# NickTravers/NeuralNetworkLibrary

Hardware: AMD Instinct MI355X
Metric: ResNet-34 224x224 training throughput (Learner.train1minibatch, fwd+loss+bwd+optimizer) (higher is better)
Workload: dtype f32; 1 GPU; DogsCats ResNet-34 classifier, 224x224, bs=64 per GPU, SGD momentum 0.9, fp32; global_batch=64, image_size=224, parallelism=dp1

## Files before the change

### include/nnl.h

```cpp
#ifndef NNL_H_
#define NNL_H_

#include <stddef.h>
#include <stdint.h>

#ifdef __cplusplus
extern "C" {
#endif

typedef enum {
  NNL_OK = 0,
  NNL_ERR_INVALID_ARG = -1,
  NNL_ERR_HIP = -2,
  NNL_ERR_UNSUPPORTED = -3,
  NNL_ERR_WORKSPACE = -4
} nnl_status_t;

int nnl_version(void);
const char* nnl_last_error(void);
int nnl_reload_env(void);

enum { NNL_PROF_CONV_FWD = 0, NNL_PROF_CONV_DGRAD = 1, NNL_PROF_CONV_WGRAD = 2, NNL_PROF_EMBDOT = 3,
       NNL_PROF_TABULAR = 4, NNL_PROF_RETINA_LOSS = 5, NNL_PROF_LSTM = 6, NNL_PROF_SOFTMAX_CE = 7,
       NNL_PROF_ELEMENTWISE = 8, NNL_PROF_GEMM = 9, NNL_PROF_OPTIM = 10, NNL_PROF_KINDS = 11 };
// ... 49 lines not shown
int nnl_wino_filter_multi(const nnl_wino_desc_t* desc, const int32_t* block_desc, int64_t n_blocks, void* stream);
int nnl_conv2d_fwd_pre(const float* x, const float* w, const float* bias, float* y, const nnl_conv_geom_t* g, int relu,
                       void* workspace, size_t workspace_bytes, int32_t* tile_counters, float* bn_partials, const float* bn_pivot,
                       int32_t* bn_rows, const float* u, void* stream);
int nnl_conv2d_dgrad_pre(const float* dy, const float* wt, float* dx, const nnl_conv_geom_t* g, const float* addend,
                         void* workspace, size_t workspace_bytes, int32_t* tile_counters, const float* u, void* stream);
size_t nnl_debug_conv_wino_workspace_bytes(int N, int H, int W, int C, int K);
int nnl_debug_conv_wino_fwd(const float* x, const float* filt, const float* bias, const float* add, float* y, void* ws,
                            size_t ws_bytes, int32_t* counters, long n_counters, float* bn_part, const float* bn_pivot, int N,
                            int H, int W, int C, int K, int relu, int flip, void* stream);
size_t nnl_debug_conv_wino2_workspace_bytes(int N, int H, int W, int C, int K);
int nnl_debug_conv_wino2_fwd(const float* x, const float* filt, const float* bias, const float* add, float* y, void* ws,
                            size_t ws_bytes, int32_t* counters, long n_counters, float* bn_part, const float* bn_pivot, int N,
                            int H, int W, int C, int K, int relu, int flip, void* stream);
int nnl_debug_conv_plan_times(int N, int H, int W, int C, int K, double* out);
size_t nnl_conv2d_wgrad_workspace_bytes(const nnl_conv_geom_t* g);
int nnl_conv2d_wgrad(const float* x, const float* dy, float* dw, const nnl_conv_geom_t* g, void* workspace,
                     size_t workspace_bytes, void* stream);
size_t nnl_colsum_workspace_bytes(int64_t rows, int64_t cols);
int nnl_sum_tensors(const float* const* src, int n, float* out, int64_t numel, void* stream);
int nnl_colsum(const float* a, float* out, int64_t rows, int64_t cols, void* workspace, size_t workspace_bytes,
               void* stream);
int nnl_relu_gate_colsum(const float* dy, const float* y, float* g, float* colsum, int64_t rows, int64_t cols, void* workspace,
                         size_t workspace_bytes, void* stream);
int nnl_act_gate_colsum(const float* dy, const float* y, float* g, float* colsum, int64_t rows, int64_t cols, int act,
                        void* workspace, size_t workspace_bytes, void* stream);

size_t nnl_bn_workspace_bytes(int64_t rows, int64_t C);
int nnl_bn_fwd(const float* x, const float* gamma, const float* beta, const float* residual, float* y,
               float* save_mean, float* save_invstd, float* running_mean, float* running_var, int64_t rows,
// ... 148 lines not shown
```

### neuralnetworklibrary_amd/_lib.py

```python
import ctypes as C
import os

import torch

_HERE = os.path.dirname(os.path.abspath(__file__))
LIB_PATH = os.environ.get('NNL_LIB_PATH') or os.path.join(_HERE, 'libnnl_hip.so')

if not os.path.exists(LIB_PATH):
    raise ImportError(
        f"{LIB_PATH} not found: build it with `python -c 'import __graft_entry__ as g; g.build()'` "
        "(or `make -C neuralnetworklibrary_amd/csrc`). There is no CPU fallback for the HIP hot path.")

lib = C.CDLL(LIB_PATH)

c_p = C.c_void_p
i32, i64, f32, f64 = C.c_int32, C.c_int64, C.c_float, C.c_double
sz = C.c_size_t


class ConvGeom(C.Structure):
    _fields_ = [('N', i32), ('H', i32), ('W', i32), ('C', i32), ('K', i32), ('R', i32), ('S', i32),
                ('stride', i32), ('pad', i32), ('P', i32), ('Q', i32)]


# ... 13 lines not shown
    'nnl_embdotbias_bwd_workspace_bytes': (sz, [i64]),
    'nnl_embdotbias_bwd': (C.c_int, [c_p, c_p, c_p, c_p, c_p, c_p, c_p, c_p, c_p, i64, i64, i64, i64, C.c_int,
                                     f32, f32, c_p, sz, c_p]),
    'nnl_conv2d_fwd_workspace_bytes': (sz, [C.POINTER(ConvGeom)]),
    'nnl_conv2d_dgrad_workspace_bytes': (sz, [C.POINTER(ConvGeom)]),
    'nnl_conv2d_tile_counters': (i64, []),
    'nnl_conv2d_wino_preferred': (C.c_int, [C.POINTER(ConvGeom), C.c_int]),
    'nnl_wino_filter_multi': (C.c_int, [c_p, c_p, i64, c_p]),
    'nnl_conv2d_fwd_pre': (C.c_int, [c_p, c_p, c_p, c_p, C.POINTER(ConvGeom), C.c_int, c_p, sz, c_p, c_p, c_p, C.POINTER(i32), c_p, c_p]),
    'nnl_conv2d_dgrad_pre': (C.c_int, [c_p, c_p, c_p, C.POINTER(ConvGeom), c_p, c_p, sz, c_p, c_p, c_p]),
    'nnl_debug_conv_wino_workspace_bytes': (sz, [C.c_int] * 5),
    'nnl_debug_conv_wino_fwd': (C.c_int, [c_p] * 6 + [sz, c_p, C.c_long, c_p, c_p] + [C.c_int] * 7 + [c_p]),
    'nnl_debug_conv_wino2_workspace_bytes': (sz, [C.c_int] * 5),
    'nnl_debug_conv_wino2_fwd': (C.c_int, [c_p] * 6 + [sz, c_p, C.c_long, c_p, c_p] + [C.c_int] * 7 + [c_p]),
    'nnl_debug_conv_plan_times': (C.c_int, [C.c_int] * 5 + [C.POINTER(C.c_double)]),
    'nnl_conv2d_fwd': (C.c_int, [c_p, c_p, c_p, c_p, C.POINTER(ConvGeom), C.c_int, c_p, sz, c_p, c_p, c_p, C.POINTER(i32), c_p]),
    'nnl_conv2d_weight_transpose': (C.c_int, [c_p, c_p, C.c_int, C.c_int, C.c_int, C.c_int, c_p]),
    'nnl_conv2d_weight_transpose_multi': (C.c_int, [c_p, c_p, i64, f64, c_p]),
    'nnl_conv2d_dgrad': (C.c_int, [c_p, c_p, c_p, C.POINTER(ConvGeom), c_p, c_p, sz, c_p, c_p]),
    'nnl_conv2d_wgrad_workspace_bytes': (sz, [C.POINTER(ConvGeom)]),
    'nnl_conv2d_wgrad': (C.c_int, [c_p, c_p, c_p, C.POINTER(ConvGeom), c_p, sz, c_p]),
    'nnl_colsum_workspace_bytes': (sz, [i64, i64]),
    'nnl_colsum': (C.c_int, [c_p, c_p, i64, i64, c_p, sz, c_p]),
    'nnl_relu_gate_colsum': (C.c_int, [c_p, c_p, c_p, c_p, i64, i64, c_p, sz, c_p]),
    'nnl_conv2d_fwd_add_up2': (C.c_int, [c_p, c_p, c_p, c_p, c_p, C.POINTER(ConvGeom), c_p]),
    'nnl_upsample2_bwd': (C.c_int, [c_p, c_p, i64, i64, i64, i64, c_p]),
    'nnl_act_gate_colsum': (C.c_int, [c_p, c_p, c_p, c_p, i64, i64, C.c_int, c_p, sz, c_p]),
    'nnl_maxpool2d_fwd': (C.c_int, [c_p, c_p, c_p, i64, i64, i64, i64, i64, i64, C.c_int, C.c_int, C.c_int, c_p]),
    'nnl_maxpool2d_bwd': (C.c_int, [c_p, c_p, c_p, i64, i64, i64, i64, i64, i64, C.c_int, C.c_int, C.c_int, c_p]),
    'nnl_sum_tensors': (C.c_int, [c_p, C.c_int, c_p, i64, c_p]),
# ... 123 lines not shown
```

### neuralnetworklibrary_amd/csrc/igemm.h

```cpp
#pragma once
#include "nnl_common.h"

typedef float f32x16 __attribute__((ext_vector_type(16)));
typedef float f32x4 __attribute__((ext_vector_type(4)));

struct IgemmRowkParams {
  const float* a;
  const float* b;
  float* y;
  const float* bias;
  const float* add;
  int N, H, W, C;
  int P, Q;
  int R, S, stride, pad;
  int M, Nc, Kg;
  int relu;
  int grid_m, grid_n;
};

struct IgemmKmajorParams {
  const float* a;
  const float* b;
  float* y;
  int N, H, W, C;
  int P, Q;
  int R, S, stride, pad;
  int Mc, Nc;
  long Kp;
  int splits, k_per_split;
  int grid_m, grid_n;
};

int nnl_internal_gemm_nt(const float* a, const float* b, float* y, const float* bias, const float* add, int M, int N,
                         int K, int relu, hipStream_t s);
int nnl_internal_gemm_nt_splitk(const float* a, const float* b, float* y_slabs, int M, int N, int K, int splits, hipStream_t s);
size_t nnl_internal_gemm_tn_workspace_bytes(int Mc, int Nc, long Kp);
int nnl_internal_gemm_tn(const float* a, const float* b, float* y, int Mc, int Nc, long Kp, void* ws, size_t ws_bytes,
                         hipStream_t s);

__device__ __forceinline__ int nnl_xcd_remap(int bid, int nblk) {
  const int q = nblk >> 3, r = nblk & 7;
  const int xcd = bid & 7, idx = bid >> 3;
  const int base = (xcd < r) ? xcd * (q + 1) : r * (q + 1) + (xcd - r) * q;
  return base + idx;
}
```

### neuralnetworklibrary_amd/csrc/wino2.hip

```cpp
#include "wino.h"
#include "wino_filter.h"
#include "igemm_taps.h"
#include <algorithm>

namespace {

constexpr int kCUs = 256;

template <int POL>
__device__ __forceinline__ f32x4 buf_load4_spol(__amdgpu_buffer_rsrc_t rsrc, unsigned voff, unsigned soff) {
  const i32x4 v = __builtin_bit_cast(i32x4, __builtin_amdgcn_raw_buffer_load_b128(rsrc, (int)voff, (int)soff, POL));
  return __builtin_bit_cast(f32x4, v);
}

struct Wino2Params {
  const float* a;
  const float* b;
  float* y;
  const float* bias;
  const float* add;
  unsigned a_bytes, b_bytes;
  int H, W, C, H2, W2;
  int ch;
  int prio;
  int M4;
  unsigned mg_W2, mg_H2;
  int Nc;
// ... 2 lines not shown
  int bal, main_ks, n_main_tiles, tail_slices, tail_row0;
  float* main_out; long main_slab_stride;
  float* tail_out; long tail_slab_stride;
  int* tile_counters;
  float* bn_part; const float* bn_pivot;
  int pos_cs;
};

__global__ void wino2_filter_kernel(const float* __restrict__ w, float* __restrict__ u, long KC, int C, int flip) {
  const long i = (long)blockIdx.x * blockDim.x + threadIdx.x;
  if (i >= KC) return;
  const long c = i % C, k = i / C;
  wino2_filter_item(w + k * 9 * C + c, u + k * 16 * C + c, C, flip);
}

template <int BK, int OCC, bool POS = false>
__global__ __launch_bounds__(256, OCC) void wino2_kernel(const Wino2Params p) {
  constexpr int BM = 64, BN = 64, BKP = BK + 4, KC = BK / 4, RPP = 256 / KC, PA = BM / RPP, PB = BN / RPP;
  __shared__ __attribute__((aligned(16))) float lds[2][(BM + BN) * BKP];
  const int tid = threadIdx.x, lane = tid & 63, wave = tid >> 6, wm = wave >> 1, wn = wave & 1;
  int logical, kslice = 0, nslices = 1, row0 = 0;
  bool in_tail = false;
  if (p.bal) {
    const int nmb = p.n_main_tiles * p.main_ks;
    if ((int)blockIdx.x < nmb) {
      const int u = nnl_xcd_remap(blockIdx.x, nmb);
      logical = u / p.main_ks;
      kslice = u - logical * p.main_ks;
      nslices = p.main_ks;
    } else {
      const int tb = (int)blockIdx.x - nmb;
      const int t = tb / p.tail_slices;
      kslice = tb - t * p.tail_slices;
      logical = p.n_main_tiles + t;
      nslices = p.tail_slices;
      if (nslices > 1) { row0 = p.tail_row0; in_tail = true; }
    }
  } else {
    logical = nnl_xcd_remap(blockIdx.x, gridDim.x);
  }
  const bool partial = nslices > 1;
  const int tile_m = logical / p.grid_n, tile_n = logical - tile_m * p.grid_n;
  const int m0 = tile_m * BM, n0 = tile_n * BN;
  const int kc = tid % KC, lrow = tid / KC;
  auto qdiv = [](int n, unsigned mg) { return mg ? (int)__umulhi((unsigned)n, mg) : n; };
  const __amdgpu_buffer_rsrc_t ra_src = __builtin_amdgcn_make_buffer_rsrc(const_cast<float*>(p.a), 0, (int)p.a_bytes, 0x00020000);
  const __amdgpu_buffer_rsrc_t rb_src = __builtin_amdgcn_make_buffer_rsrc(const_cast<float*>(p.b), 0, (int)p.b_bytes, 0x00020000);

  int a_off[PA];
  unsigned rmask[PA], cmask[PA];
#pragma unroll
  for (int i = 0; i < PA; ++i) {
    const int m = m0 + lrow + i * RPP;
    const bool valid = m < p.M4;
    const int mm = valid ? m : 0;
    const int l2 = qdiv(mm, p.mg_W2), j = mm - l2 * p.W2;
    const int n = qdiv(l2, p.mg_H2), ii = l2 - n * p.H2;
    a_off[i] = (((n * p.H + 2 * ii - 1) * p.W + 2 * j - 1) * p.C + kc * 4) * 4;
    unsigned rm = 0, cm = 0;
    if (valid) {
      for (int a = 0; a < 4; ++a) if ((unsigned)(2 * ii - 1 + a) < (unsigned)p.H) rm |= 1u << a;
      for (int a = 0; a < 4; ++a) if ((unsigned)(2 * j - 1 + a) < (unsigned)p.W) cm |= 1u << a;
    }
    rmask[i] = rm; cmask[i] = cm;
  }
  unsigned b_off[PB];
#pragma unroll
  for (int i = 0; i < PB; ++i) {
    const int nr = n0 + lrow + i * RPP;
    b_off[i] = nr < p.Nc ? (unsigned)(nr * 16 * p.C + kc * 4) * 4u : 0xFFFFFFFFu;
  }
  unsigned v00[PA], v01[PA], v10[PA], v11[PA], b_tap = 0;
  float sr = 1.f, sc = 1.f;
  auto set_pos = [&](int t) {
    const int xi = t >> 2, nu = t & 3;
    const int ra_ = xi, rb_ = xi < 2 ? 2 : 1;
    const int ca = nu, cb = nu < 2 ? 2 : 1;
    sr = xi == 1 ? 1.f : -1.f;
    sc = nu == 1 ? 1.f : -1.f;
    b_tap = (unsigned)(t * p.C) * 4u;
    const int wc = p.W * p.C * 4, c4 = p.C * 4;
#pragma unroll
    for (int i = 0; i < PA; ++i) {
      const bool ra_ok = (rmask[i] >> ra_) & 1u, rb_ok = (rmask[i] >> rb_) & 1u;
      const bool ca_ok = (cmask[i] >> ca) & 1u, cb_ok = (cmask[i] >> cb) & 1u;
      v00[i] = (ra_ok && ca_ok) ? (unsigned)(a_off[i] + ra_ * wc + ca * c4) : 0xFFFFFFFFu;
// ... 15 lines not shown
  float sr_ld = 1.f, sc_ld = 1.f;
  auto store_tile = [&](int buf) {
    float* As = lds[buf];
    float* Bs = As + BM * BKP;
#pragma unroll
    for (int i = 0; i < PA; ++i) {
      f32x4 v;
#pragma unroll
      for (int e = 0; e < 4; ++e)
        v[e] = __builtin_fmaf(sr_ld, __builtin_fmaf(sc_ld, r11[i][e], r10[i][e]), __builtin_fmaf(sc_ld, r01[i][e], r00[i][e]));
      *reinterpret_cast<f32x4*>(As + (lrow + i * RPP) * BKP + kc * 4) = v;
    }
#pragma unroll
    for (int i = 0; i < PB; ++i) *reinterpret_cast<f32x4*>(Bs + (lrow + i * RPP) * BKP + kc * 4) = rb[i];
  };
  const int frag_off = (lane & 31) * BKP + (lane >> 5) * 4;
  auto compute = [&](int buf, f32x16& acc) {
    const float* As = lds[buf] + wm * 32 * BKP + frag_off;
    const float* Bs = lds[buf] + BM * BKP + wn * 32 * BKP + frag_off;
    f32x4 fa[BK / 8], fb[BK / 8];
#pragma unroll
    for (int kk = 0; kk < BK / 8; ++kk) {
      fa[kk] = *reinterpret_cast<const f32x4*>(As + kk * 8);
      fb[kk] = *reinterpret_cast<const f32x4*>(Bs + kk * 8);
    }
#pragma unroll
    for (int kk = 0; kk < BK / 8; ++kk)
#pragma unroll
      for (int t = 0; t < 4; ++t) acc = __builtin_amdgcn_mfma_f32_32x32x2f32(fa[kk][t], fb[kk][t], acc, 0, 0, 0);
  };

  f32x16 y00, y01, y10, y11, tm;
#pragma unroll
  for (int e = 0; e < 16; ++e) { tm[e] = 0.f; }
  if constexpr (!POS) {
#pragma unroll
    for (int e = 0; e < 16; ++e) { y00[e] = 0.f; y01[e] = 0.f; y10[e] = 0.f; y11[e] = 0.f; }
  }
  const int csteps = p.C / BK, nk_all = 16 * csteps, cpc = p.ch / BK, per_chunk = 16 * cpc;
  if constexpr (POS) {
    const int t_pos = kslice / p.pos_cs, sub = kslice - t_pos * p.pos_cs, nkb = csteps / p.pos_cs;
    set_pos(t_pos);
    sr_ld = sr; sc_ld = sc;
    const int cb0 = sub * nkb * BK;
    load_tile(cb0);
    store_tile(0);
    __syncthreads();
    int cur = 0;
    for (int kt = 0; kt < nkb; ++kt) {
      if (kt + 1 < nkb) load_tile(cb0 + (kt + 1) * BK);
      __builtin_amdgcn_sched_barrier(0);
      compute(cur, tm);
      __builtin_amdgcn_sched_barrier(0);
      if (kt + 1 < nkb) store_tile(cur ^ 1);
      __syncthreads();
      cur ^= 1;
    }
  }
  int kt0 = 0, nk = nk_all;
  if (POS) nk = 0;
  else if (partial) {
    const int per = (nk_all + nslices - 1) / nslices;
    kt0 = kslice * per;
    nk = min(per, nk_all - kt0);
    if (nk < 0) nk = 0;
  }
  const int kend = kt0 + nk;
  int chunk_nx = kt0 / per_chunk, t_nx = (kt0 - chunk_nx * per_chunk) / cpc, cs_nx = kt0 - chunk_nx * per_chunk - t_nx * cpc;
  int c_nx = chunk_nx * p.ch + cs_nx * BK;
  int t_cur = t_nx, cs_cur = cs_nx;
  auto advance = [&]() {
    if (++cs_nx == cpc) {
      cs_nx = 0;
      if (++t_nx == 16) { t_nx = 0; ++chunk_nx; }
      set_pos(t_nx);
    }
// ... 35 lines not shown
      }
      if (k10 != 0.f) {
#pragma unroll
        for (int e = 0; e < 16; ++e) y10[e] = __builtin_fmaf(k10, tm[e], y10[e]);
      }
      if (k11 != 0.f) {
#pragma unroll
        for (int e = 0; e < 16; ++e) y11[e] = __builtin_fmaf(k11, tm[e], y11[e]);
      }
#pragma unroll
      for (int e = 0; e < 16; ++e) tm[e] = 0.f;
      cs_cur = 0; t_cur = (t_cur + 1) & 15;
    }
  }

  const int col_l = lane & 31, row_h = (lane >> 5) * 4;
  constexpr int kSc1 = 1 << 4;
  if constexpr (POS) {
    __shared__ int ticket;
    const long sstride = p.main_slab_stride;
    const __amdgpu_buffer_rsrc_t rs = __builtin_amdgcn_make_buffer_rsrc(p.main_out, 0, (int)((long)nslices * sstride * 4), 0x00020000);
    const int cl = n0 + wn * 32 + col_l;
#pragma unroll
    for (int e = 0; e < 16; ++e) {
      const int row = m0 + wm * 32 + (e & 3) + 8 * (e >> 2) + row_h;
      const long off = (long)kslice * sstride + (long)row * p.Nc + cl;
      const bool ok = row < p.M4 && cl < p.Nc;
      __builtin_amdgcn_raw_buffer_store_b32(__float_as_uint(tm[e]), rs, ok ? (int)(off * 4) : -1, 0, kSc1);
    }
    asm volatile("s_waitcnt vmcnt(0)" ::: "memory");
    __syncthreads();
    if (tid == 0) ticket = __hip_atomic_fetch_add(&p.tile_counters[logical], 1, __ATOMIC_RELAXED, __HIP_MEMORY_SCOPE_AGENT);
    __syncthreads();
    if (ticket != nslices - 1) return;
    if (tid == 0) __hip_atomic_store(&p.tile_counters[logical], 0, __ATOMIC_RELAXED, __HIP_MEMORY_SCOPE_AGENT);
    float fs1[4] = {0.f, 0.f, 0.f, 0.f}, fs2[4] = {0.f, 0.f, 0.f, 0.f};
    const int c4 = n0 + (tid & 15) * 4, cs = p.pos_cs;
    const int wrow = p.W * p.Nc;
    auto item_off = [&](int k4, bool& ok) {
      const int row = m0 + (tid >> 4) + 16 * k4;
      ok = row < p.M4 && c4 < p.Nc;
      return ok ? (unsigned)(((long)row * p.Nc + c4) * 4) : 0xFFFFFFFFu;
    };
    auto finish_item = [&](int k4, f32x4 (&m)[16]) {
      const int row = m0 + (tid >> 4) + 16 * k4;
      f32x4 r0[4], r1[4];
#pragma unroll
      for (int xi = 0; xi < 4; ++xi) {
        r0[xi] = (m[xi * 4 + 0] + m[xi * 4 + 1]) + m[xi * 4 + 2];
        r1[xi] = (m[xi * 4 + 1] - m[xi * 4 + 2]) + m[xi * 4 + 3];
      }
      f32x4 out[4];
      out[0] = (r0[0] + r0[1]) + r0[2];
      out[1] = (r1[0] + r1[1]) + r1[2];
      out[2] = (r0[1] - r0[2]) + r0[3];
      out[3] = (r1[1] - r1[2]) + r1[3];
      const int l2 = qdiv(row, p.mg_W2), j = row - l2 * p.W2;
      const int n = qdiv(l2, p.mg_H2), ii = l2 - n * p.H2;
      const long ob = (((long)n * p.H + 2 * ii) * p.W + 2 * j) * p.Nc + c4;
      const bool h1 = 2 * ii + 1 < p.H, w1 = 2 * j + 1 < p.W;
#pragma unroll
      for (int h = 0; h < 4; ++h) {
        if (((h >> 1) && !h1) || ((h & 1) && !w1)) continue;
        f32x4 v = out[h];
        const long o = ob + (h >> 1) * wrow + (h & 1) * p.Nc;
        if (p.bias) v += *reinterpret_cast<const f32x4*>(p.bias + c4);
        if (p.add) v += *reinterpret_cast<const f32x4*>(p.add + o);
        if (p.relu == 1) { v[0] = fmaxf(v[0], 0.f); v[1] = fmaxf(v[1], 0.f); v[2] = fmaxf(v[2], 0.f); v[3] = fmaxf(v[3], 0.f); }
        *reinterpret_cast<f32x4*>(p.y + o) = v;
        if (p.bn_part) {
          const f32x4 pv = *reinterpret_cast<const f32x4*>(p.bn_pivot + c4);
#pragma unroll
          for (int e = 0; e < 4; ++e) { const float d = v[e] - pv[e]; fs1[e] += d; fs2[e] += d * d; }
        }
      }
    };
#pragma unroll 1
    for (int k4 = 0; k4 < 4; ++k4) {
      bool ok_a;
      const unsigned oa = item_off(k4, ok_a);
      if (!ok_a) continue;
      f32x4 ma[16];
#pragma unroll
      for (int t = 0; t < 16; ++t) ma[t] = buf_load4_spol<kSc1>(rs, oa, (unsigned)((long)(t * cs) * sstride * 4));
      for (int sl = 1; sl < cs; ++sl) {
#pragma unroll
        for (int t0 = 0; t0 < 16; t0 += 8) {
          f32x4 pa[8];
#pragma unroll
          for (int t = 0; t < 8; ++t) pa[t] = buf_load4_spol<kSc1>(rs, oa, (unsigned)((long)((t0 + t) * cs + sl) * sstride * 4));
#pragma unroll
          for (int t = 0; t < 8; ++t) ma[t0 + t] += pa[t];
        }
      }
      finish_item(k4, ma);
    }
    if (p.bn_part) {
      __syncthreads();
      float* red = &lds[0][0];
#pragma unroll
      for (int e = 0; e < 4; ++e) {
        red[(((tid >> 4) * 64) + (tid & 15) * 4 + e) * 2 + 0] = fs1[e];
        red[(((tid >> 4) * 64) + (tid & 15) * 4 + e) * 2 + 1] = fs2[e];
      }
      __syncthreads();
      if (tid < 64 && n0 + tid < p.Nc) {
        float a = 0.f, b = 0.f;
        for (int r = 0; r < 16; ++r) { a += red[(r * 64 + tid) * 2]; b += red[(r * 64 + tid) * 2 + 1]; }
        p.bn_part[((long)tile_m * p.Nc + n0 + tid) * 2 + 0] = a;
        p.bn_part[((long)tile_m * p.Nc + n0 + tid) * 2 + 1] = b;
      }
    }
    return;
  }
  if (partial) {
    __shared__ int ticket;
    float* const base = in_tail ? p.tail_out : p.main_out;
    const long sstride = in_tail ? p.tail_slab_stride : p.main_slab_stride;
    const __amdgpu_buffer_rsrc_t rs = __builtin_amdgcn_make_buffer_rsrc(base, 0, (int)((long)nslices * sstride * 4), 0x00020000);
    const int cl = n0 + wn * 32 + col_l;
#pragma unroll
    for (int e = 0; e < 16; ++e) {
      const int row = m0 + wm * 32 + (e & 3) + 8 * (e >> 2) + row_h;
      const long off = (long)kslice * sstride + (long)(row - row0) * 4 * p.Nc + cl;
      const bool ok = row < p.M4 && cl < p.Nc;
      __builtin_amdgcn_raw_buffer_store_b32(__float_as_uint(y00[e]), rs, ok ? (int)(off * 4) : -1, 0, kSc1);
      __builtin_amdgcn_raw_buffer_store_b32(__float_as_uint(y01[e]), rs, ok ? (int)((off + p.Nc) * 4) : -1, 0, kSc1);
      __builtin_amdgcn_raw_buffer_store_b32(__float_as_uint(y10[e]), rs, ok ? (int)((off + 2 * p.Nc) * 4) : -1, 0, kSc1);
      __builtin_amdgcn_raw_buffer_store_b32(__float_as_uint(y11[e]), rs, ok ? (int)((off + 3 * p.Nc) * 4) : -1, 0, kSc1);
// ... 102 lines not shown
    __syncthreads();
    if (tid < 64 && n0 + tid < p.Nc) {
      float a = 0.f, b = 0.f;
      for (int r = 0; r < 16; ++r) { a += red[(r * 64 + tid) * 2]; b += red[(r * 64 + tid) * 2 + 1]; }
      p.bn_part[((long)tile_m * p.Nc + n0 + tid) * 2 + 0] = a;
      p.bn_part[((long)tile_m * p.Nc + n0 + tid) * 2 + 1] = b;
    }
  }
}

struct W2Plan {
  int bk, on, main_ks, n_main_tiles, tail_slices, tail_row0;
  size_t main_floats, tail_floats;
  double t_us;
  int pos_cs;
};

double w2_pos_cost(long T, long M4, int Nc, int C, int cs) {
  const double a = 0.363, b = 0.490, tfix = 4.0;
  const long occ = 4, nwg = T * 16 * cs, I = (C / 32) / cs;
  const long nb = nnl_cdiv(nwg, (long)kCUs);
  const double c = (double)(nb < occ ? nb : occ);
  const double slab_b = 2.0 * 16 * cs * (double)M4 * Nc * 4;
  return nb * I * (b + a / c) + tfix * nb / c + slab_b / 11.7e6 + (3.0 + 1.5 * cs) + 4.0;
}

double w2_cost(long T, long gn, long M4, int Nc, long I, int bk, int ks, int S, W2Plan* out) {
  const double a = bk == 32 ? 0.363 : 0.226, b = bk == 32 ? 0.490 : 0.243, tfix = bk == 32 ? 12.3 : 15.0;
  const long occ = bk == 16 ? 4 : 3;
  long n_main = ((T * ks / kCUs) * kCUs / ks / gn) * gn;
  if (n_main > T) n_main = T;
  const long tail = T - n_main;
  if (tail == 0 && S > 1) return -1.0;
  const long m = nnl_cdiv(n_main * ks, (long)kCUs), q = nnl_cdiv(tail * S, (long)kCUs);
  const long W = m * nnl_cdiv(I, (long)ks) + q * nnl_cdiv(I, (long)S), nb = m + q;
  const double c = (double)(nb < occ ? nb : occ);
  const long row0 = (n_main / gn) * 64 < M4 ? (n_main / gn) * 64 : M4;
  const double main_b = ks > 1 ? (2.0 * ks + 1) * row0 * 4 * Nc * 4 : 0;
  const double tail_b = (S > 1 && tail) ? (2.0 * S + 1) * (M4 - row0) * 4 * Nc * 4 : 0;
// ... 24 lines not shown
        W2Plan cand{};
        const double t = w2_cost(T, gn, M4, Nc, I, bk, ks, S, &cand);
        if (t < 0) break;
        if (f_S > 0 && balance && cand.n_main_tiles < T && S != f_S) continue;
        if (t < best_t) { best_t = t; best = cand; best.t_us = t; }
      }
    }
  }
  if (best_t == 1e300) {
    best.t_us = w2_cost(T, gn, M4, Nc, 16L * (C / 16), 16, 1, 1, &best);
    best_t = best.t_us;
  }
  const int e_pos = NNL_ENV_INT("NNL_WINO2_POS", -1);
  if (e_pos != 0 && (balance || e_pos > 0) && C % 32 == 0) {
    const int csteps = C / 32;
    double pt = 1e300; int pcs = 0;
    for (int cs = 1; cs <= 8; cs *= 2) {
      if (csteps % cs != 0 || (csteps / cs < 2 && cs > 1)) break;
      if (e_pos > 0 && cs != e_pos && csteps % e_pos == 0) continue;
      const size_t fl = (size_t)16 * cs * M4 * Nc;
      if (fl * sizeof(float) >= (1UL << 31)) break;
      const double t = w2_pos_cost(T, M4, Nc, C, cs);
      if (t < pt) { pt = t; pcs = cs; }
    }
    if (pcs && (e_pos > 0 || pt < best_t)) {
      best = W2Plan{};
      best.bk = 32; best.on = 1; best.main_ks = 16 * pcs; best.n_main_tiles = (int)T; best.tail_slices = 1; best.tail_row0 = (int)M4;
      best.main_floats = (size_t)16 * pcs * M4 * Nc; best.tail_floats = 0; best.t_us = pt; best.pos_cs = pcs;
    }
  }
  return best;
}

size_t align4(size_t floats) { return (floats + 3) & ~(size_t)3; }

long quads(int N, int H, int W) { return (long)N * ((H + 1) / 2) * ((W + 1) / 2); }

}

bool nnl_wino2_ok(int N, int H, int W, int Cin, int Nc, int R, int S, int stride, int pad) {
  if (R != 3 || S != 3 || stride != 1 || pad != 1 || W < 2 || H < 2 || Cin % 16 != 0 || Nc % 4 != 0) return false;
  const long a_b = (long)N * H * W * Cin * 4, b_b = (long)Nc * 16 * Cin * 4, y_b = (long)N * H * W * Nc * 4;
  if ((quads(N, H, W) + 128) * (long)std::max((W + 1) / 2, (H + 1) / 2) >= (1L << 32)) return false;
// ... 38 lines not shown
  const long T = (long)p.grid_m * p.grid_n;
  W2Plan pl = wino2_plan(M4, q.Nc, q.Cin);
  if (pl.on && (tile_counters == nullptr || T > n_counters || ws_bytes < (u_floats + pl.main_floats + pl.tail_floats) * sizeof(float) ||
                pl.main_floats * sizeof(float) >= (1UL << 31) || pl.tail_floats * sizeof(float) >= (1UL << 31))) {
    if (pl.pos_cs) {
      const int bk = q.Cin % 32 == 0 ? 32 : 16;
      w2_cost(T, p.grid_n, M4, q.Nc, 16L * (q.Cin / bk), bk, 1, 1, &pl);
      pl.pos_cs = 0;
    }
    pl.on = 0;
  }
  unsigned grid = (unsigned)T;
  if (pl.pos_cs) {
    p.bal = 1; p.main_ks = pl.main_ks; p.n_main_tiles = pl.n_main_tiles; p.tail_slices = 1; p.tail_row0 = (int)M4;
    p.main_out = u + u_floats; p.main_slab_stride = M4 * q.Nc; p.tile_counters = tile_counters; p.pos_cs = pl.pos_cs;
    grid = (unsigned)(T * pl.main_ks);
    hipLaunchKernelGGL((wino2_kernel<32, 4, true>), dim3(grid), dim3(256), 0, s, p);
    NNL_CHECK_LAUNCH();
    return NNL_OK;
  }
  if (pl.on) {
    p.bal = 1; p.main_ks = pl.main_ks; p.n_main_tiles = pl.n_main_tiles; p.tail_slices = pl.tail_slices; p.tail_row0 = pl.tail_row0;
    p.main_out = u + u_floats; p.main_slab_stride = (long)pl.tail_row0 * 4 * q.Nc;
    p.tail_out = p.main_out + pl.main_floats; p.tail_slab_stride = (long)(M4 - pl.tail_row0) * 4 * q.Nc;
    p.tile_counters = tile_counters;
    grid = (unsigned)(pl.n_main_tiles * pl.main_ks + (T - pl.n_main_tiles) * pl.tail_slices);
  }
  if (pl.bk == 32) hipLaunchKernelGGL((wino2_kernel<32, 3>), dim3(grid), dim3(256), 0, s, p);
  else hipLaunchKernelGGL((wino2_kernel<16, 4>), dim3(grid), dim3(256), 0, s, p);
  NNL_CHECK_LAUNCH();
  return NNL_OK;
}

extern "C" size_t nnl_debug_conv_wino2_workspace_bytes(int N, int H, int W, int C, int K) { return nnl_wino2_workspace_bytes(N, H, W, C, K); }
extern "C" int nnl_debug_conv_wino2_fwd(const float* x, const float* w, const float* bias, const float* add, float* y, void* ws,
                                        size_t ws_bytes, int32_t* counters, long n_counters, float* bn_part, const float* bn_pivot, int N,
                                        int H, int W, int C, int K, int relu, int flip, void* stream) {
  NNL_CHECK_ARG(nnl_wino2_ok(N, H, W, C, K, 3, 3, 1, 1), "wino2: unsupported shape");
  WinoProblem q{};
  q.in = x; q.filt = w; q.out = y; q.bias = bias; q.add = add; q.N = N; q.H = H; q.W = W; q.Cin = C; q.Nc = K; q.relu = relu; q.flip = flip;
  q.bn_part = bn_part; q.bn_pivot = bn_pivot;
  return nnl_wino2_launch(q, ws, ws_bytes, counters, n_counters, (hipStream_t)stream);
}
```

Baseline: 5552 images/s.

## Add persistent-grid scheduling for wino2 position-split kernel with cross-item prefetch

Adds a persistent variant of the position-split Winograd F(2,3) kernel. A fixed grid of 4 workgroups per CU walks a contiguous, XCD-aware range of (tile, slice) work items and prefetches the next item's first K-tile while finishing the current one. The last slice to arrive does the reduction and output transform. The planner picks the persistent grid when its cost model beats the one-block-per-item launch and the item count divides evenly by the grid size. The aim is to cut per-workgroup launch and prologue overhead and tail imbalance, at the cost of more complex control flow and register pressure. A debug schedule-dump entry point is also added.

```diff
diff --git a/include/nnl.h b/include/nnl.h
--- a/include/nnl.h
+++ b/include/nnl.h
@@ -87,6 +87,7 @@
                             size_t ws_bytes, int32_t* counters, long n_counters, float* bn_part, const float* bn_pivot, int N,
                             int H, int W, int C, int K, int relu, int flip, void* stream);
 int nnl_debug_conv_plan_times(int N, int H, int W, int C, int K, double* out);
+int64_t nnl_debug_wino2_schedule(int N, int H, int W, int C, int K, int64_t* hdr, int64_t* rows, int64_t cap);
 size_t nnl_conv2d_wgrad_workspace_bytes(const nnl_conv_geom_t* g);
 int nnl_conv2d_wgrad(const float* x, const float* dy, float* dw, const nnl_conv_geom_t* g, void* workspace,
                      size_t workspace_bytes, void* stream);
diff --git a/neuralnetworklibrary_amd/_lib.py b/neuralnetworklibrary_amd/_lib.py
--- a/neuralnetworklibrary_amd/_lib.py
+++ b/neuralnetworklibrary_amd/_lib.py
@@ -51,6 +51,7 @@
     'nnl_debug_conv_wino2_workspace_bytes': (sz, [C.c_int] * 5),
     'nnl_debug_conv_wino2_fwd': (C.c_int, [c_p] * 6 + [sz, c_p, C.c_long, c_p, c_p] + [C.c_int] * 7 + [c_p]),
     'nnl_debug_conv_plan_times': (C.c_int, [C.c_int] * 5 + [C.POINTER(C.c_double)]),
+    'nnl_debug_wino2_schedule': (i64, [C.c_int] * 5 + [C.POINTER(i64), C.POINTER(i64), i64]),
     'nnl_conv2d_fwd': (C.c_int, [c_p, c_p, c_p, c_p, C.POINTER(ConvGeom), C.c_int, c_p, sz, c_p, c_p, c_p, C.POINTER(i32), c_p]),
     'nnl_conv2d_weight_transpose': (C.c_int, [c_p, c_p, C.c_int, C.c_int, C.c_int, C.c_int, c_p]),
     'nnl_conv2d_weight_transpose_multi': (C.c_int, [c_p, c_p, i64, f64, c_p]),
diff --git a/neuralnetworklibrary_amd/csrc/igemm.h b/neuralnetworklibrary_amd/csrc/igemm.h
--- a/neuralnetworklibrary_amd/csrc/igemm.h
+++ b/neuralnetworklibrary_amd/csrc/igemm.h
@@ -38,7 +38,7 @@
 int nnl_internal_gemm_tn(const float* a, const float* b, float* y, int Mc, int Nc, long Kp, void* ws, size_t ws_bytes,
                          hipStream_t s);
 
-__device__ __forceinline__ int nnl_xcd_remap(int bid, int nblk) {
+__host__ __device__ __forceinline__ int nnl_xcd_remap(int bid, int nblk) {
   const int q = nblk >> 3, r = nblk & 7;
   const int xcd = bid & 7, idx = bid >> 3;
   const int base = (xcd < r) ? xcd * (q + 1) : r * (q + 1) + (xcd - r) * q;
diff --git a/neuralnetworklibrary_amd/csrc/wino2.hip b/neuralnetworklibrary_amd/csrc/wino2.hip
--- a/neuralnetworklibrary_amd/csrc/wino2.hip
+++ b/neuralnetworklibrary_amd/csrc/wino2.hip
@@ -11,6 +11,15 @@
 __device__ __forceinline__ f32x4 buf_load4_spol(__amdgpu_buffer_rsrc_t rsrc, unsigned voff, unsigned soff) {
   const i32x4 v = __builtin_bit_cast(i32x4, __builtin_amdgcn_raw_buffer_load_b128(rsrc, (int)voff, (int)soff, POL));
   return __builtin_bit_cast(f32x4, v);
+}
+
+__host__ __device__ inline void w2_pos_range(int bid, int G, int total, int* it, int* it_end) {
+  const int q = total / G, r = total - q * G, xcd = bid & 7, idx = bid >> 3;
+  const int nl = (r >> 3) + (xcd < (r & 7) ? 1 : 0);
+  const int before_x = xcd * (r >> 3) + (xcd < (r & 7) ? xcd : (r & 7));
+  const int u = nnl_xcd_remap(bid, G);
+  *it = u * q + before_x + (idx < nl ? idx : nl);
+  *it_end = *it + q + (idx < nl ? 1 : 0);
 }
 
 struct Wino2Params {
@@ -43,14 +52,24 @@
   wino2_filter_item(w + k * 9 * C + c, u + k * 16 * C + c, C, flip);
 }
 
-template <int BK, int OCC, bool POS = false>
+template <int BK, int OCC, bool POS = false, bool PERSIST = false>
 __global__ __launch_bounds__(256, OCC) void wino2_kernel(const Wino2Params p) {
   constexpr int BM = 64, BN = 64, BKP = BK + 4, KC = BK / 4, RPP = 256 / KC, PA = BM / RPP, PB = BN / RPP;
   __shared__ __attribute__((aligned(16))) float lds[2][(BM + BN) * BKP];
-  const int tid = threadIdx.x, lane = tid & 63, wave = tid >> 6, wm = wave >> 1, wn = wave & 1;
+  int tid = threadIdx.x, lane = tid & 63, wave = tid >> 6, wm = wave >> 1, wn = wave & 1;
   int logical, kslice = 0, nslices = 1, row0 = 0;
   bool in_tail = false;
-  if (p.bal) {
+  int it = 0, it_end = 0;
+  if constexpr (POS) {
+    nslices = p.main_ks;
+    if constexpr (PERSIST) {
+      w2_pos_range((int)blockIdx.x, (int)gridDim.x, p.n_main_tiles * nslices, &it, &it_end);
+    } else {
+      it = nnl_xcd_remap(blockIdx.x, gridDim.x);
+      it_end = it + 1;
+    }
+    logical = it / nslices;
+  } else if (p.bal) {
     const int nmb = p.n_main_tiles * p.main_ks;
     if ((int)blockIdx.x < nmb) {
       const int u = nnl_xcd_remap(blockIdx.x, nmb);
@@ -71,34 +90,37 @@
   const bool partial = nslices > 1;
   const int tile_m = logical / p.grid_n, tile_n = logical - tile_m * p.grid_n;
   const int m0 = tile_m * BM, n0 = tile_n * BN;
-  const int kc = tid % KC, lrow = tid / KC;
+  int kc = tid % KC, lrow = tid / KC;
   auto qdiv = [](int n, unsigned mg) { return mg ? (int)__umulhi((unsigned)n, mg) : n; };
   const __amdgpu_buffer_rsrc_t ra_src = __builtin_amdgcn_make_buffer_rsrc(const_cast<float*>(p.a), 0, (int)p.a_bytes, 0x00020000);
   const __amdgpu_buffer_rsrc_t rb_src = __builtin_amdgcn_make_buffer_rsrc(const_cast<float*>(p.b), 0, (int)p.b_bytes, 0x00020000);
 
   int a_off[PA];
   unsigned rmask[PA], cmask[PA];
-#pragma unroll
-  for (int i = 0; i < PA; ++i) {
-    const int m = m0 + lrow + i * RPP;
-    const bool valid = m < p.M4;
-    const int mm = valid ? m : 0;
-    const int l2 = qdiv(mm, p.mg_W2), j = mm - l2 * p.W2;
-    const int n = qdiv(l2, p.mg_H2), ii = l2 - n * p.H2;
-    a_off[i] = (((n * p.H + 2 * ii - 1) * p.W + 2 * j - 1) * p.C + kc * 4) * 4;
-    unsigned rm = 0, cm = 0;
-    if (valid) {
-      for (int a = 0; a < 4; ++a) if ((unsigned)(2 * ii - 1 + a) < (unsigned)p.H) rm |= 1u << a;
-      for (int a = 0; a < 4; ++a) if ((unsigned)(2 * j - 1 + a) < (unsigned)p.W) cm |= 1u << a;
-    }
-    rmask[i] = rm; cmask[i] = cm;
-  }
   unsigned b_off[PB];
-#pragma unroll
-  for (int i = 0; i < PB; ++i) {
-    const int nr = n0 + lrow + i * RPP;
-    b_off[i] = nr < p.Nc ? (unsigned)(nr * 16 * p.C + kc * 4) * 4u : 0xFFFFFFFFu;
-  }
+  auto set_tile = [&](int tm0, int tn0) {
+#pragma unroll
+    for (int i = 0; i < PA; ++i) {
+      const int m = tm0 + lrow + i * RPP;
+      const bool valid = m < p.M4;
+      const int mm = valid ? m : 0;
+      const int l2 = qdiv(mm, p.mg_W2), j = mm - l2 * p.W2;
+      const int n = qdiv(l2, p.mg_H2), ii = l2 - n * p.H2;
+      a_off[i] = (((n * p.H + 2 * ii - 1) * p.W + 2 * j - 1) * p.C + kc * 4) * 4;
+      unsigned rm = 0, cm = 0;
+      if (valid) {
+        for (int a = 0; a < 4; ++a) if ((unsigned)(2 * ii - 1 + a) < (unsigned)p.H) rm |= 1u << a;
+        for (int a = 0; a < 4; ++a) if ((unsigned)(2 * j - 1 + a) < (unsigned)p.W) cm |= 1u << a;
+      }
+      rmask[i] = rm; cmask[i] = cm;
+    }
+#pragma unroll
+    for (int i = 0; i < PB; ++i) {
+      const int nr = tn0 + lrow + i * RPP;
+      b_off[i] = nr < p.Nc ? (unsigned)(nr * 16 * p.C + kc * 4) * 4u : 0xFFFFFFFFu;
+    }
+  };
+  if constexpr (!POS) set_tile(m0, n0);
   unsigned v00[PA], v01[PA], v10[PA], v11[PA], b_tap = 0;
   float sr = 1.f, sc = 1.f;
   auto set_pos = [&](int t) {
@@ -144,10 +166,11 @@
 #pragma unroll
     for (int i = 0; i < PB; ++i) *reinterpret_cast<f32x4*>(Bs + (lrow + i * RPP) * BKP + kc * 4) = rb[i];
   };
-  const int frag_off = (lane & 31) * BKP + (lane >> 5) * 4;
+  int frag_off = (lane & 31) * BKP + (lane >> 5) * 4;
+  int frag_a = wm * 32 * BKP + frag_off, frag_b = BM * BKP + wn * 32 * BKP + frag_off;
   auto compute = [&](int buf, f32x16& acc) {
-    const float* As = lds[buf] + wm * 32 * BKP + frag_off;
-    const float* Bs = lds[buf] + BM * BKP + wn * 32 * BKP + frag_off;
+    const float* As = lds[buf] + (POS ? frag_a : wm * 32 * BKP + frag_off);
+    const float* Bs = lds[buf] + (POS ? frag_b : BM * BKP + wn * 32 * BKP + frag_off);
     f32x4 fa[BK / 8], fb[BK / 8];
 #pragma unroll
     for (int kk = 0; kk < BK / 8; ++kk) {
@@ -168,28 +191,168 @@
     for (int e = 0; e < 16; ++e) { y00[e] = 0.f; y01[e] = 0.f; y10[e] = 0.f; y11[e] = 0.f; }
   }
   const int csteps = p.C / BK, nk_all = 16 * csteps, cpc = p.ch / BK, per_chunk = 16 * cpc;
+  int col_l = lane & 31, row_h = (lane >> 5) * 4;
+  constexpr int kSc1 = 1 << 4;
   if constexpr (POS) {
-    const int t_pos = kslice / p.pos_cs, sub = kslice - t_pos * p.pos_cs, nkb = csteps / p.pos_cs;
-    set_pos(t_pos);
-    sr_ld = sr; sc_ld = sc;
-    const int cb0 = sub * nkb * BK;
-    load_tile(cb0);
-    store_tile(0);
-    __syncthreads();
-    int cur = 0;
-    for (int kt = 0; kt < nkb; ++kt) {
-      if (kt + 1 < nkb) load_tile(cb0 + (kt + 1) * BK);
-      __builtin_amdgcn_sched_barrier(0);
-      compute(cur, tm);
-      __builtin_amdgcn_sched_barrier(0);
-      if (kt + 1 < nkb) store_tile(cur ^ 1);
+    __shared__ int pos_ticket;
+    const int nkb = csteps / p.pos_cs;
+    const long sstride = p.main_slab_stride;
+    const __amdgpu_buffer_rsrc_t rs = __builtin_amdgcn_make_buffer_rsrc(p.main_out, 0, (int)((long)nslices * sstride * 4), 0x00020000);
+    const int wrow = p.W * p.Nc;
+    int cb = 0;
+    auto setup_item = [&](int item) {
+      item = __builtin_amdgcn_readfirstlane(item);
+      const int tile = item / nslices, ks = item - tile * nslices;
+      const int tmi = tile / p.grid_n, tni = tile - tmi * p.grid_n;
+      set_tile(tmi * BM, tni * BN);
+      const int t_pos = ks / p.pos_cs, sub = ks - t_pos * p.pos_cs;
+      set_pos(t_pos);
+      cb = sub * nkb * BK;
+    };
+    auto publish_item = [&](int item) -> bool {
+      item = __builtin_amdgcn_readfirstlane(item);
+      const int tile = item / nslices, ks = item - tile * nslices;
+      const int tmi = tile / p.grid_n, tni = tile - tmi * p.grid_n;
+      const int im0 = tmi * BM, in0 = tni * BN;
+      const int cl = in0 + wn * 32 + col_l;
+#pragma unroll
+      for (int e = 0; e < 16; ++e) {
+        const int row = im0 + wm * 32 + (e & 3) + 8 * (e >> 2) + row_h;
+        const long off = (long)ks * sstride + (long)row * p.Nc + cl;
+        const bool ok = row < p.M4 && cl < p.Nc;
+        __builtin_amdgcn_raw_buffer_store_b32(__float_as_uint(tm[e]), rs, ok ? (int)(off * 4) : -1, 0, kSc1);
+      }
+      asm volatile("s_waitcnt vmcnt(0)" ::: "memory");
       __syncthreads();
-      cur ^= 1;
-    }
+      if (tid == 0) pos_ticket = __hip_atomic_fetch_add(&p.tile_counters[tile], 1, __ATOMIC_RELAXED, __HIP_MEMORY_SCOPE_AGENT);
+      __syncthreads();
+      return __builtin_amdgcn_readfirstlane(pos_ticket) == nslices - 1;
+    };
+    auto reduce_tile = [&](int item, float* red) {
+      item = __builtin_amdgcn_readfirstlane(item);
+      const int tile = item / nslices;
+      const int tmi = tile / p.grid_n, tni = tile - tmi * p.grid_n;
+      const int im0 = tmi * BM, in0 = tni * BN;
+      if (tid == 0) __hip_atomic_store(&p.tile_counters[tile], 0, __ATOMIC_RELAXED, __HIP_MEMORY_SCOPE_AGENT);
+      float fs1[4] = {0.f, 0.f, 0.f, 0.f}, fs2[4] = {0.f, 0.f, 0.f, 0.f};
+      const int c4 = in0 + (tid & 15) * 4, cs = p.pos_cs;
+      constexpr int NB = 8, XR = 4;
+#pragma unroll 1
+      for (int k4 = 0; k4 < 4; ++k4) {
+        const int row = im0 + (tid >> 4) + 16 * k4;
+        if (!(row < p.M4 && c4 < p.Nc)) continue;
+        const unsigned oa = (unsigned)(((long)row * p.Nc + c4) * 4);
+        f32x4 r0[4], r1[4];
+#pragma unroll
+        for (int x0 = 0; x0 < 4; x0 += XR) {
+          f32x4 m[XR * 4];
+#pragma unroll
+          for (int t = 0; t < XR * 4; ++t) m[t] = buf_load4_spol<kSc1>(rs, oa, (unsigned)((long)((x0 * 4 + t) * cs) * sstride * 4));
+          for (int sl = 1; sl < cs; ++sl) {
+#pragma unroll
+            for (int t0 = 0; t0 < XR * 4; t0 += NB) {
+              f32x4 pa[NB];
+#pragma unroll
+              for (int t = 0; t < NB; ++t) pa[t] = buf_load4_spol<kSc1>(rs, oa, (unsigned)((long)((x0 * 4 + t0 + t) * cs + sl) * sstride * 4));
+#pragma unroll
+              for (int t = 0; t < NB; ++t) m[t0 + t] += pa[t];
+            }
+          }
+#pragma unroll
+          for (int xi = 0; xi < XR; ++xi) {
+            r0[x0 + xi] = (m[xi * 4 + 0] + m[xi * 4 + 1]) + m[xi * 4 + 2];
+            r1[x0 + xi] = (m[xi * 4 + 1] - m[xi * 4 + 2]) + m[xi * 4 + 3];
+          }
+        }
+        f32x4 out[4];
+        out[0] = (r0[0] + r0[1]) + r0[2];
+        out[1] = (r1[0] + r1[1]) + r1[2];
+        out[2] = (r0[1] - r0[2]) + r0[3];
+        out[3] = (r1[1] - r1[2]) + r1[3];
+        const int l2 = qdiv(row, p.mg_W2), j = row - l2 * p.W2;
+        const int n = qdiv(l2, p.mg_H2), ii = l2 - n * p.H2;
+        const long ob = (((long)n * p.H + 2 * ii) * p.W + 2 * j) * p.Nc + c4;
+        const bool h1 = 2 * ii + 1 < p.H, w1 = 2 * j + 1 < p.W;
+#pragma unroll
+        for (int h = 0; h < 4; ++h) {
+          if (((h >> 1) && !h1) || ((h & 1) && !w1)) continue;
+          f32x4 v = out[h];
+          const long o = ob + (h >> 1) * wrow + (h & 1) * p.Nc;
+          if (p.bias) v += *reinterpret_cast<const f32x4*>(p.bias + c4);
+          if (p.add) v += *reinterpret_cast<const f32x4*>(p.add + o);
+          if (p.relu == 1) { v[0] = fmaxf(v[0], 0.f); v[1] = fmaxf(v[1], 0.f); v[2] = fmaxf(v[2], 0.f); v[3] = fmaxf(v[3], 0.f); }
+          *reinterpret_cast<f32x4*>(p.y + o) = v;
+          if (p.bn_part) {
+            const f32x4 pv = *reinterpret_cast<const f32x4*>(p.bn_pivot + c4);
+#pragma unroll
+            for (int e = 0; e < 4; ++e) { const float d = v[e] - pv[e]; fs1[e] += d; fs2[e] += d * d; }
+          }
+        }
+      }
+      if (p.bn_part) {
+#pragma unroll
+        for (int e = 0; e < 4; ++e) {
+          red[(((tid >> 4) * 64) + (tid & 15) * 4 + e) * 2 + 0] = fs1[e];
+          red[(((tid >> 4) * 64) + (tid & 15) * 4 + e) * 2 + 1] = fs2[e];
+        }
+        __syncthreads();
+        if (tid < 64 && in0 + tid < p.Nc) {
+          float a = 0.f, b = 0.f;
+          for (int r = 0; r < 16; ++r) { a += red[(r * 64 + tid) * 2]; b += red[(r * 64 + tid) * 2 + 1]; }
+          p.bn_part[((long)tmi * p.Nc + in0 + tid) * 2 + 0] = a;
+          p.bn_part[((long)tmi * p.Nc + in0 + tid) * 2 + 1] = b;
+        }
+        __syncthreads();
+      }
+    };
+    int nkb_o = nkb;
+    asm volatile("" : "+s"(nkb_o));
+    int item = it;
+    while (item < it_end) {
+      if constexpr (PERSIST) {
+        asm volatile("" : "+v"(tid));
+        lane = tid & 63; wave = tid >> 6; wm = wave >> 1; wn = wave & 1; kc = tid % KC; lrow = tid / KC;
+        frag_off = (lane & 31) * BKP + (lane >> 5) * 4; col_l = lane & 31; row_h = (lane >> 5) * 4;
+        frag_a = wm * 32 * BKP + frag_off; frag_b = BM * BKP + wn * 32 * BKP + frag_off;
+      }
+      setup_item(item);
+      sr_ld = sr; sc_ld = sc;
+      load_tile(cb);
+      store_tile(0);
+      __syncthreads();
+      int cur = 0, red_item = -1;
+      for (;;) {
+        const int cb0 = __builtin_amdgcn_readfirstlane(cb);
+        for (int kt = 0; kt + 1 < nkb; ++kt) {
+          load_tile(cb0 + (kt + 1) * BK);
+          __builtin_amdgcn_sched_barrier(0);
+          compute(cur, tm);
+          __builtin_amdgcn_sched_barrier(0);
+          if (kt + 1 < nkb_o) store_tile(cur ^ 1);
+          __syncthreads();
+          cur ^= 1;
+        }
+        const bool more = PERSIST && item + 1 < it_end;
+        if (more) { setup_item(item + 1); load_tile(cb); }
+        __builtin_amdgcn_sched_barrier(0);
+        compute(cur, tm);
+        __builtin_amdgcn_sched_barrier(0);
+        if (more) { sr_ld = sr; sc_ld = sc; store_tile(cur ^ 1); }
+        __syncthreads();
+        cur ^= 1;
+        const bool last = publish_item(item);
+#pragma unroll
+        for (int e = 0; e < 16; ++e) tm[e] = 0.f;
+        ++item;
+        if (last) { red_item = item - 1; break; }
+        if (!more) break;
+      }
+      if (red_item >= 0) reduce_tile(red_item, &lds[0][0]);
+    }
+    return;
   }
   int kt0 = 0, nk = nk_all;
-  if (POS) nk = 0;
-  else if (partial) {
+  if (partial) {
     const int per = (nk_all + nslices - 1) / nslices;
     kt0 = kslice * per;
     nk = min(per, nk_all - kt0);
@@ -255,105 +418,6 @@
     }
   }
 
-  const int col_l = lane & 31, row_h = (lane >> 5) * 4;
-  constexpr int kSc1 = 1 << 4;
-  if constexpr (POS) {
-    __shared__ int ticket;
-    const long sstride = p.main_slab_stride;
-    const __amdgpu_buffer_rsrc_t rs = __builtin_amdgcn_make_buffer_rsrc(p.main_out, 0, (int)((long)nslices * sstride * 4), 0x00020000);
-    const int cl = n0 + wn * 32 + col_l;
-#pragma unroll
-    for (int e = 0; e < 16; ++e) {
-      const int row = m0 + wm * 32 + (e & 3) + 8 * (e >> 2) + row_h;
-      const long off = (long)kslice * sstride + (long)row * p.Nc + cl;
-      const bool ok = row < p.M4 && cl < p.Nc;
-      __builtin_amdgcn_raw_buffer_store_b32(__float_as_uint(tm[e]), rs, ok ? (int)(off * 4) : -1, 0, kSc1);
-    }
-    asm volatile("s_waitcnt vmcnt(0)" ::: "memory");
-    __syncthreads();
-    if (tid == 0) ticket = __hip_atomic_fetch_add(&p.tile_counters[logical], 1, __ATOMIC_RELAXED, __HIP_MEMORY_SCOPE_AGENT);
-    __syncthreads();
-    if (ticket != nslices - 1) return;
-    if (tid == 0) __hip_atomic_store(&p.tile_counters[logical], 0, __ATOMIC_RELAXED, __HIP_MEMORY_SCOPE_AGENT);
-    float fs1[4] = {0.f, 0.f, 0.f, 0.f}, fs2[4] = {0.f, 0.f, 0.f, 0.f};
-    const int c4 = n0 + (tid & 15) * 4, cs = p.pos_cs;
-    const int wrow = p.W * p.Nc;
-    auto item_off = [&](int k4, bool& ok) {
-      const int row = m0 + (tid >> 4) + 16 * k4;
-      ok = row < p.M4 && c4 < p.Nc;
-      return ok ? (unsigned)(((long)row * p.Nc + c4) * 4) : 0xFFFFFFFFu;
-    };
-    auto finish_item = [&](int k4, f32x4 (&m)[16]) {
-      const int row = m0 + (tid >> 4) + 16 * k4;
-      f32x4 r0[4], r1[4];
-#pragma unroll
-      for (int xi = 0; xi < 4; ++xi) {
-        r0[xi] = (m[xi * 4 + 0] + m[xi * 4 + 1]) + m[xi * 4 + 2];
-        r1[xi] = (m[xi * 4 + 1] - m[xi * 4 + 2]) + m[xi * 4 + 3];
-      }
-      f32x4 out[4];
-      out[0] = (r0[0] + r0[1]) + r0[2];
-      out[1] = (r1[0] + r1[1]) + r1[2];
-      out[2] = (r0[1] - r0[2]) + r0[3];
-      out[3] = (r1[1] - r1[2]) + r1[3];
-      const int l2 = qdiv(row, p.mg_W2), j = row - l2 * p.W2;
-      const int n = qdiv(l2, p.mg_H2), ii = l2 - n * p.H2;
-      const long ob = (((long)n * p.H + 2 * ii) * p.W + 2 * j) * p.Nc + c4;
-      const bool h1 = 2 * ii + 1 < p.H, w1 = 2 * j + 1 < p.W;
-#pragma unroll
-      for (int h = 0; h < 4; ++h) {
-        if (((h >> 1) && !h1) || ((h & 1) && !w1)) continue;
-        f32x4 v = out[h];
-        const long o = ob + (h >> 1) * wrow + (h & 1) * p.Nc;
-        if (p.bias) v += *reinterpret_cast<const f32x4*>(p.bias + c4);
-        if (p.add) v += *reinterpret_cast<const f32x4*>(p.add + o);
-        if (p.relu == 1) { v[0] = fmaxf(v[0], 0.f); v[1] = fmaxf(v[1], 0.f); v[2] = fmaxf(v[2], 0.f); v[3] = fmaxf(v[3], 0.f); }
-        *reinterpret_cast<f32x4*>(p.y + o) = v;
-        if (p.bn_part) {
-          const f32x4 pv = *reinterpret_cast<const f32x4*>(p.bn_pivot + c4);
-#pragma unroll
-          for (int e = 0; e < 4; ++e) { const float d = v[e] - pv[e]; fs1[e] += d; fs2[e] += d * d; }
-        }
-      }
-    };
-#pragma unroll 1
-    for (int k4 = 0; k4 < 4; ++k4) {
-      bool ok_a;
-      const unsigned oa = item_off(k4, ok_a);
-      if (!ok_a) continue;
-      f32x4 ma[16];
-#pragma unroll
-      for (int t = 0; t < 16; ++t) ma[t] = buf_load4_spol<kSc1>(rs, oa, (unsigned)((long)(t * cs) * sstride * 4));
-      for (int sl = 1; sl < cs; ++sl) {
-#pragma unroll
-        for (int t0 = 0; t0 < 16; t0 += 8) {
-          f32x4 pa[8];
-#pragma unroll
-          for (int t = 0; t < 8; ++t) pa[t] = buf_load4_spol<kSc1>(rs, oa, (unsigned)((long)((t0 + t) * cs + sl) * sstride * 4));
-#pragma unroll
-          for (int t = 0; t < 8; ++t) ma[t0 + t] += pa[t];
-        }
-      }
-      finish_item(k4, ma);
-    }
-    if (p.bn_part) {
-      __syncthreads();
-      float* red = &lds[0][0];
-#pragma unroll
-      for (int e = 0; e < 4; ++e) {
-        red[(((tid >> 4) * 64) + (tid & 15) * 4 + e) * 2 + 0] = fs1[e];
-        red[(((tid >> 4) * 64) + (tid & 15) * 4 + e) * 2 + 1] = fs2[e];
-      }
-      __syncthreads();
-      if (tid < 64 && n0 + tid < p.Nc) {
-        float a = 0.f, b = 0.f;
-        for (int r = 0; r < 16; ++r) { a += red[(r * 64 + tid) * 2]; b += red[(r * 64 + tid) * 2 + 1]; }
-        p.bn_part[((long)tile_m * p.Nc + n0 + tid) * 2 + 0] = a;
-        p.bn_part[((long)tile_m * p.Nc + n0 + tid) * 2 + 1] = b;
-      }
-    }
-    return;
-  }
   if (partial) {
     __shared__ int ticket;
     float* const base = in_tail ? p.tail_out : p.main_out;
@@ -486,6 +550,7 @@
   size_t main_floats, tail_floats;
   double t_us;
   int pos_cs;
+  int pos_grid;
 };
 
 double w2_pos_cost(long T, long M4, int Nc, int C, int cs) {
@@ -495,6 +560,15 @@
   const double c = (double)(nb < occ ? nb : occ);
   const double slab_b = 2.0 * 16 * cs * (double)M4 * Nc * 4;
   return nb * I * (b + a / c) + tfix * nb / c + slab_b / 11.7e6 + (3.0 + 1.5 * cs) + 4.0;
+}
+
+constexpr double kPosItemUs = 2.25;
+double w2_pos_persist_cost(long T, long M4, int Nc, int C, int cs) {
+  const double a = 0.363, b = 0.490, c = 4.0;
+  const long G = kCUs * 4, items = T * 16 * cs, I = (C / 32) / cs;
+  const long ni = 4 * (items / G) + std::min(4L, nnl_cdiv(items % G, (long)kCUs));
+  const double slab_b = 2.0 * 16 * cs * (double)M4 * Nc * 4;
+  return ni * I * (b + a / c) + kPosItemUs * ni / c + slab_b / 11.7e6 + (3.0 + 1.5 * cs) + 4.0;
 }
 
 double w2_cost(long T, long gn, long M4, int Nc, long I, int bk, int ks, int S, W2Plan* out) {
@@ -549,19 +623,26 @@
   const int e_pos = NNL_ENV_INT("NNL_WINO2_POS", -1);
   if (e_pos != 0 && (balance || e_pos > 0) && C % 32 == 0) {
     const int csteps = C / 32;
-    double pt = 1e300; int pcs = 0;
+    const int e_per = NNL_ENV_INT("NNL_WINO2_PERSIST", -1);
+    double pt = 1e300; int pcs = 0, pgrid = 0;
     for (int cs = 1; cs <= 8; cs *= 2) {
       if (csteps % cs != 0 || (csteps / cs < 2 && cs > 1)) break;
       if (e_pos > 0 && cs != e_pos && csteps % e_pos == 0) continue;
       const size_t fl = (size_t)16 * cs * M4 * Nc;
       if (fl * sizeof(float) >= (1UL << 31)) break;
-      const double t = w2_pos_cost(T, M4, Nc, C, cs);
-      if (t < pt) { pt = t; pcs = cs; }
+      const long items = T * 16 * cs;
+      double t = w2_pos_cost(T, M4, Nc, C, cs);
+      int g = (int)items;
+      if (e_per != 0 && balance && items > kCUs * 4) {
+        const double tp = w2_pos_persist_cost(T, M4, Nc, C, cs);
+        if (e_per > 0 || (tp < t && items % (kCUs * 4) == 0)) { t = tp; g = kCUs * 4; }
+      }
+      if (t < pt) { pt = t; pcs = cs; pgrid = g; }
     }
     if (pcs && (e_pos > 0 || pt < best_t)) {
       best = W2Plan{};
       best.bk = 32; best.on = 1; best.main_ks = 16 * pcs; best.n_main_tiles = (int)T; best.tail_slices = 1; best.tail_row0 = (int)M4;
-      best.main_floats = (size_t)16 * pcs * M4 * Nc; best.tail_floats = 0; best.t_us = pt; best.pos_cs = pcs;
+      best.main_floats = (size_t)16 * pcs * M4 * Nc; best.tail_floats = 0; best.t_us = pt; best.pos_cs = pcs; best.pos_grid = pgrid;
     }
   }
   return best;
@@ -630,8 +711,9 @@
   if (pl.pos_cs) {
     p.bal = 1; p.main_ks = pl.main_ks; p.n_main_tiles = pl.n_main_tiles; p.tail_slices = 1; p.tail_row0 = (int)M4;
     p.main_out = u + u_floats; p.main_slab_stride = M4 * q.Nc; p.tile_counters = tile_counters; p.pos_cs = pl.pos_cs;
-    grid = (unsigned)(T * pl.main_ks);
-    hipLaunchKernelGGL((wino2_kernel<32, 4, true>), dim3(grid), dim3(256), 0, s, p);
+    grid = (unsigned)pl.pos_grid;
+    if (pl.pos_grid < T * pl.main_ks) hipLaunchKernelGGL((wino2_kernel<32, 4, true, true>), dim3(grid), dim3(256), 0, s, p);
+    else hipLaunchKernelGGL((wino2_kernel<32, 4, true>), dim3(grid), dim3(256), 0, s, p);
     NNL_CHECK_LAUNCH();
     return NNL_OK;
   }
@@ -646,6 +728,74 @@
   else hipLaunchKernelGGL((wino2_kernel<16, 4>), dim3(grid), dim3(256), 0, s, p);
   NNL_CHECK_LAUNCH();
   return NNL_OK;
+}
+
+extern "C" int64_t nnl_debug_wino2_schedule(int N, int H, int W, int C, int K, int64_t* hdr, int64_t* rows, int64_t cap) {
+  if (!nnl_wino2_ok(N, H, W, C, K, 3, 3, 1, 1) || hdr == nullptr) return -1;
+  const long M4 = quads(N, H, W), gm = nnl_cdiv(M4, 64L), gn = nnl_cdiv(K, 64), T = gm * gn;
+  const W2Plan pl = wino2_plan(M4, K, C);
+  const long u_floats = (long)align4((size_t)K * 16 * C), I = 16L * (C / pl.bk);
+  const bool split = pl.on != 0;
+  long grid = T;
+  if (pl.pos_cs) grid = pl.pos_grid;
+  else if (split) grid = (long)pl.n_main_tiles * pl.main_ks + (T - pl.n_main_tiles) * pl.tail_slices;
+  for (int i = 0; i < 16; ++i) hdr[i] = 0;
+  hdr[0] = pl.pos_cs ? 2 : (split ? 1 : 0); hdr[1] = grid; hdr[2] = pl.bk; hdr[3] = (pl.pos_cs || pl.bk == 16) ? 4 : 3; hdr[4] = T; hdr[5] = I;
+  hdr[6] = pl.pos_cs; hdr[7] = pl.pos_cs && grid < T * pl.main_ks; hdr[8] = (int64_t)nnl_wino2_workspace_bytes(N, H, W, C, K);
+  hdr[9] = pl.pos_cs ? T * pl.main_ks : 0; hdr[10] = pl.main_ks; hdr[11] = pl.n_main_tiles; hdr[12] = pl.tail_slices; hdr[13] = kCUs;
+  int64_t n = 0;
+  auto emit = [&](long wg, long tile, long slice, long nsl, long k0, long k1, long lo, long hi) {
+    if (rows && n < cap) {
+      int64_t* r = rows + n * 8;
+      r[0] = wg; r[1] = tile; r[2] = slice; r[3] = nsl; r[4] = k0; r[5] = k1; r[6] = lo; r[7] = hi;
+    }
+    ++n;
+  };
+  auto rows_of = [&](long tile, long& m0, long& m1, long& n0, long& n1) {
+    const long tm = tile / gn, tn = tile - tm * gn;
+    m0 = tm * 64; m1 = std::min(m0 + 64, M4); n0 = tn * 64; n1 = std::min(n0 + 64, (long)K);
+  };
+  if (pl.pos_cs) {
+    const long nsl = pl.main_ks, total = T * nsl, G = grid, nkb = (C / 32) / pl.pos_cs, ss = M4 * K;
+    for (long b = 0; b < G; ++b) {
+      int it, it_end;
+      if (G < total) w2_pos_range((int)b, (int)G, (int)total, &it, &it_end);
+      else { it = nnl_xcd_remap((int)b, (int)G); it_end = it + 1; }
+      for (long item = it; item < it_end; ++item) {
+        const long tile = item / nsl, ks = item - tile * nsl;
+        long m0, m1, n0, n1;
+        rows_of(tile, m0, m1, n0, n1);
+        emit(b, tile, ks, nsl, ks * nkb, (ks + 1) * nkb, u_floats + ks * ss + m0 * K + n0, u_floats + ks * ss + (m1 - 1) * K + n1);
+      }
+    }
+    return n;
+  }
+  for (long b = 0; b < grid; ++b) {
+    long tile, ks = 0, nsl = 1, row0 = 0, base = u_floats, ss = 0;
+    if (split) {
+      const long nmb = (long)pl.n_main_tiles * pl.main_ks;
+      if (b < nmb) {
+        const long u = nnl_xcd_remap((int)b, (int)nmb);
+        tile = u / pl.main_ks; ks = u - tile * pl.main_ks; nsl = pl.main_ks; ss = (long)pl.tail_row0 * 4 * K;
+      } else {
+        const long tb = b - nmb, t = tb / pl.tail_slices;
+        ks = tb - t * pl.tail_slices; tile = pl.n_main_tiles + t; nsl = pl.tail_slices;
+        if (nsl > 1) { row0 = pl.tail_row0; base = u_floats + (long)pl.main_floats; ss = (M4 - pl.tail_row0) * 4 * K; }
+      }
+    } else {
+      tile = nnl_xcd_remap((int)b, (int)grid);
+    }
+    long k0 = 0, k1 = I, lo = -1, hi = -1;
+    if (nsl > 1) {
+      const long per = (I + nsl - 1) / nsl;
+      k0 = ks * per; k1 = std::max(k0, std::min(k0 + per, I));
+      long m0, m1, n0, n1;
+      rows_of(tile, m0, m1, n0, n1);
+      lo = base + ks * ss + (m0 - row0) * 4 * K + n0; hi = base + ks * ss + ((m1 - 1 - row0) * 4 + 3) * K + n1;
+    }
+    emit(b, tile, ks, nsl, k0, k1, lo, hi);
+  }
+  return n;
 }
 
 extern "C" size_t nnl_debug_conv_wino2_workspace_bytes(int N, int H, int W, int C, int K) { return nnl_wino2_workspace_bytes(N, H, W, C, K); }
```

Result: faster. 5611 images/s, median of 6 (+1.1%).
